# carkod/binquant

Measured on AMD Instinct MI355X. Metric: symbol-candles/s for full indicator set (14 fp64 columns), higher is better.
Workload: dtype f64; 1 GPU; configs[3]: 100000 symbols x 10000 candles, symbol-sharded over 1 GPU(s) (100000 symbols x 10000 candles on rank 0); symbols=100000, symbols_per_gpu=100000, candles=10000, parallelism=symbol-sharded x1, no data-path collective

## Files before the change

binquant_amd/csrc/bq_enrich.hip:

```cpp
#include "bq_device.h"
#include "binquant_amd.h"

#include <stddef.h>
#include <string.h>

#include <type_traits>

namespace bq {

#ifndef BQ_EN_NT
#define BQ_EN_NT 256
#endif
#ifndef BQ_EN_K
#define BQ_EN_K 4
#endif
#ifndef BQ_EN_NTSTORE
#define BQ_EN_NTSTORE 1
#endif
#ifndef BQ_EN_SWIZZLE
#define BQ_EN_SWIZZLE 0
#endif
#ifndef BQ_EN_WPS
#define BQ_EN_WPS 3
#endif
constexpr int EN_NT = BQ_EN_NT;
constexpr int EN_NW = EN_NT / WAVE;
constexpr int EN_K = BQ_EN_K;
constexpr int EN_TT = EN_NT * EN_K;
constexpr int EN_LK = EN_K == 2 ? 1 : EN_K == 4 ? 2 : 3;
constexpr int EN_H = 128;
constexpr int EN_R = EN_H + EN_TT;
static_assert(EN_K % 2 == 0 && EN_TT >= EN_H && EN_K * WAVE > BQ_MAX_WINDOW, "tile shape");

#ifndef BQ_EN_LDSPERM
#define BQ_EN_LDSPERM 1
#endif
#if BQ_EN_LDSPERM
#define LX(i) ((((i) & (EN_K - 1)) * (EN_R / EN_K)) + ((i) >> EN_LK))
#define RS(x) (lb + LX(x))
#define RS1(x) (pb / EN_K + LX(x))
#else
#define LX(i) (i)
#define RS(x) (pb + (x))
#define RS1(x) (pb + (x))
#endif
static_assert(!BQ_EN_LDSPERM || ((1 << EN_LK) == EN_K && EN_R % EN_K == 0), "LX: power-of-two candles per lane");

enum { E_FAST = 0, E_SLOW, E_SIG, E_0, E_1, NE };

struct Pow {
  double a0, a1, p, q, a2, a3, a4;
};

__host__ __device__ __forceinline__ Pow pow_mul(const Pow& T, const Pow& U) {
  Pow r;
  r.a0 = T.a0 * U.a0;
  r.a1 = T.a1 * U.a1;
  r.p = fma(T.p, U.a0, T.a2 * U.p);
  r.q = fma(T.q, U.a1, T.a2 * U.q);
  r.a2 = T.a2 * U.a2;
  r.a3 = T.a3 * U.a3;
  r.a4 = T.a4 * U.a4;
  return r;
}

struct EmaHost {
  double al[NE], om[NE], den[NE], la[NE], lb[NE];
  Pow step;
  Pow wstep[6];
  Pow wave[EN_NW + 1];
};

struct EnrichArgs {
  EmaHost ema;
  const double* in[BQ_NUM_INPUTS];
  double* out[BQ_NUM_ENRICH_COLS];
  int64_t ld_in, ld_out;
  int64_t S, swz;
  int T;
  int ma[3];
  int rsi_w, bb_w, bb_ddof, atr_w, twap_w, mfi_w;
  int span[NE];
  double bb_k;
  double inv_ma[3], inv_rsi, inv_bb, inv_bb_dv, inv_atr, inv_twap;
};

struct EmaConsts {
  double al[NE], om[NE], den[NE], la[NE], lb[NE];
  Pow step;
  Pow wstep[6];
  Pow wave[EN_NW + 1];
  Pow lane[WAVE];
};
static_assert(sizeof(EmaHost) % sizeof(double) == 0 && offsetof(EmaConsts, lane) == sizeof(EmaHost),
              "EmaConsts begins with EmaHost's layout");

static EmaHost ema_consts(const int (&span)[NE]) {
  EmaHost E;
  for (int e = 0; e < NE; ++e) {
    const double com = ((double)span[e] - 1.0) / 2.0;
    const double al = 1.0 / (1.0 + com);
    E.al[e] = al;
    E.om[e] = 1.0 - al;
    E.den[e] = E.om[e] + al;
    E.la[e] = E.om[e] / E.den[e];
    E.lb[e] = al / E.den[e];
  }
  Pow m;
  m.a0 = E.la[E_FAST];
  m.a1 = E.la[E_SLOW];
  m.a2 = E.la[E_SIG];
  m.p = E.lb[E_SIG] * E.la[E_FAST];
  m.q = -(E.lb[E_SIG] * E.la[E_SLOW]);
  m.a3 = E.la[E_0];
  m.a4 = E.la[E_1];
  E.step = m;
  Pow mk = m;
  for (int k = 1; k < EN_K; ++k) mk = pow_mul(m, mk);
  for (int j = 0; j < 6; ++j) {
    E.wstep[j] = mk;
    mk = pow_mul(mk, mk);
  }
  Pow r = {1.0, 1.0, 0.0, 0.0, 1.0, 1.0, 1.0};
  const Pow w64 = pow_mul(E.wstep[5], E.wstep[5]);
  for (int k = 0; k <= EN_NW; ++k) {
    E.wave[k] = r;
    r = pow_mul(w64, r);
  }
  return E;
}

__device__ __forceinline__ void pow_apply(const Pow& A, const double (&v)[NE], double (&r)[NE]) {
  r[E_FAST] = A.a0 * v[E_FAST];
  r[E_SLOW] = A.a1 * v[E_SLOW];
  r[E_SIG] = fma(A.p, v[E_FAST], fma(A.q, v[E_SLOW], A.a2 * v[E_SIG]));
  r[E_0] = A.a3 * v[E_0];
  r[E_1] = A.a4 * v[E_1];
}

template <bool DIV>
__device__ __forceinline__ double ema_step(double y, double x, const EmaConsts& E, int e) {
  if (y != x) {
    y = E.om[e] * y + E.al[e] * x;
    if (DIV) y = y / E.den[e];
  }
  return y;
}

typedef double dbl2 __attribute__((ext_vector_type(2)));

__device__ __forceinline__ void load4(const double* __restrict__ row, int tb, int T, bool vec, double (&x)[EN_K]) {
  if (vec && tb + EN_K <= T) {
    const dbl2* p = reinterpret_cast<const dbl2*>(row + tb);
#pragma unroll
    for (int j = 0; j < EN_K / 2; ++j) {
      const dbl2 a = p[j];
      x[2 * j] = a.x;
      x[2 * j + 1] = a.y;
    }
  } else {
#pragma unroll
    for (int k = 0; k < EN_K; ++k) x[k] = (tb + k < T) ? row[tb + k] : 0.0;
  }
}

typedef __attribute__((address_space(1))) double gdouble;
typedef __attribute__((address_space(1))) dbl2 gdbl2;

#ifndef BQ_EN_SWAPST
#define BQ_EN_SWAPST 1
#endif

__device__ __forceinline__ void put2(gdouble* row, int t, int T, bool full, dbl2 v) {
  if (full || t + 2 <= T) {
#if BQ_EN_NTSTORE
    __builtin_nontemporal_store(v, reinterpret_cast<gdbl2*>(row + t));
#else
    *reinterpret_cast<gdbl2*>(row + t) = v;
#endif
  } else if (t < T) {
    row[t] = v.x;
  }
}

__device__ __forceinline__ void store4(double* __restrict__ row_, int tb, int T, bool vec, const double (&x)[EN_K],
                                       bool full = false) {
  gdouble* row = (gdouble*)row_;
#if BQ_EN_SWAPST
  if constexpr (EN_K == 4) {
    if (vec) {
      union {
        dbl2 d;
        unsigned u[4];
      } a, b;
      a.d = dbl2{x[0], x[1]};
      b.d = dbl2{x[2], x[3]};
#pragma unroll
      for (int i = 0; i < 4; ++i) {
        const auto r = __builtin_amdgcn_permlane32_swap(a.u[i], b.u[i], false, false);
        a.u[i] = r[0];
        b.u[i] = r[1];
      }
      const int lane = __lane_id();
      const int ta = lane < 32 ? tb : tb - 126;
      put2(row, ta, T, full, a.d);
      put2(row, ta + 128, T, full, b.d);
      return;
    }
  }
#endif
  if (vec && tb + EN_K <= T) {
    gdbl2* p = reinterpret_cast<gdbl2*>(row + tb);
#pragma unroll
    for (int j = 0; j < EN_K / 2; ++j) {
#if BQ_EN_NTSTORE
      __builtin_nontemporal_store(dbl2{x[2 * j], x[2 * j + 1]}, p + j);
#else
      p[j] = dbl2{x[2 * j], x[2 * j + 1]};
#endif
    }
  } else {
#pragma unroll
    for (int k = 0; k < EN_K; ++k)
      if (tb + k < T) row[tb + k] = x[k];
  }
}

struct Tile {
  double o[EN_K], h[EN_K], l[EN_K], c[EN_K], v[EN_K];
  double ph, pl, pc;
};

#ifndef BQ_EN_LINELOAD
#define BQ_EN_LINELOAD 0
#endif

__device__ __forceinline__ void load_tile(const EnrichArgs& A, int64_t row, int tb, bool vin, Tile& t) {
  const int T = A.T;
  if (BQ_EN_LINELOAD && vin) {
    load_pieces<EN_K>(A.in[BQ_OPEN] + row, tb, T, t.o, 0.0);
    load_pieces<EN_K>(A.in[BQ_HIGH] + row, tb, T, t.h, 0.0);
    load_pieces<EN_K>(A.in[BQ_LOW] + row, tb, T, t.l, 0.0);
    load_pieces<EN_K>(A.in[BQ_CLOSE] + row, tb, T, t.c, 0.0);
    load_pieces<EN_K>(A.in[BQ_VOLUME] + row, tb, T, t.v, 0.0);
  } else {
    load4(A.in[BQ_OPEN] + row, tb, T, vin, t.o);
    load4(A.in[BQ_HIGH] + row, tb, T, vin, t.h);
    load4(A.in[BQ_LOW] + row, tb, T, vin, t.l);
    load4(A.in[BQ_CLOSE] + row, tb, T, vin, t.c);
    load4(A.in[BQ_VOLUME] + row, tb, T, vin, t.v);
  }
  if (tb >= 1 && tb <= T) {
    t.ph = A.in[BQ_HIGH][row + tb - 1];
    t.pl = A.in[BQ_LOW][row + tb - 1];
    t.pc = A.in[BQ_CLOSE][row + tb - 1];
  } else {
    t.ph = t.pl = t.pc = qnan();
  }
}

__device__ __forceinline__ void tile_arrived(bool vin, Tile& t) {
  if (BQ_EN_LINELOAD && vin) {
    line_unexchange_x<EN_K>(t.o);
    line_unexchange_x<EN_K>(t.h);
    line_unexchange_x<EN_K>(t.l);
    line_unexchange_x<EN_K>(t.c);
    line_unexchange_x<EN_K>(t.v);
  }
}

typedef dbl2 __attribute__((aligned(8))) dbl2u;

__device__ __forceinline__ void load_tile_clamped(const EnrichArgs& A, int64_t row, int tb, Tile& t) {
  const int T = A.T;
  int64_t u[EN_K / 2];
#pragma unroll
  for (int j = 0; j < EN_K / 2; ++j) u[j] = row + min(tb + 2 * j, T - 2);
  auto field = [&](const double* __restrict__ f, double (&x)[EN_K]) {
#pragma unroll
    for (int j = 0; j < EN_K / 2; ++j) {
      const dbl2u a = *reinterpret_cast<const dbl2u*>(f + u[j]);
      x[2 * j] = a.x;
      x[2 * j + 1] = a.y;
    }
  };
  field(A.in[BQ_OPEN], t.o);
  field(A.in[BQ_HIGH], t.h);
  field(A.in[BQ_LOW], t.l);
  field(A.in[BQ_CLOSE], t.c);
  field(A.in[BQ_VOLUME], t.v);
  const int64_t n = row + min(tb - 1, T - 1);
  t.ph = A.in[BQ_HIGH][n];
  t.pl = A.in[BQ_LOW][n];
  t.pc = A.in[BQ_CLOSE][n];
}

__device__ __forceinline__ void tile_tail_select(int tb, int T, Tile& t) {
  auto field = [&](double (&x)[EN_K]) {
#pragma unroll
    for (int j = 0; j < EN_K / 2; ++j) {
      const int u = tb + 2 * j;
      const bool both = u + 2 <= T, one = u < T;
      x[2 * j] = both ? x[2 * j] : (one ? x[2 * j + 1] : 0.0);
      x[2 * j + 1] = both ? x[2 * j + 1] : 0.0;
    }
  };
  field(t.o);
  field(t.h);
  field(t.l);
  field(t.c);
  field(t.v);
  if (tb > T) t.ph = t.pl = t.pc = qnan();
}

template <bool GEN_, bool WARM_, bool RANGE_, bool PREF_, bool SEL_>
struct TileMode {
  static constexpr bool GEN = GEN_, WARM = WARM_, RANGE = RANGE_, PREF = PREF_, SEL = SEL_;
};

template <bool DEF>
__device__ __forceinline__ int win_of(int def, int v) {
  return DEF ? def : __builtin_amdgcn_readfirstlane(v);
}

struct WinAgg {
  double sum, first;
  bool ok, same;
};

template <typename F>
__device__ __forceinline__ WinAgg win_agg(F val, int t, int w) {
  WinAgg a = {0.0, 0.0, t >= w - 1, true};
  if (!a.ok) return a;
  a.first = val(t - w + 1);
  for (int j = t - w + 1; j <= t; ++j) {
    const double x = val(j);
    if (!__builtin_isfinite(x)) {
      a.ok = false;
      return a;
    }
    a.same &= x == a.first;
    a.sum += x;
  }
  return a;
}

__device__ __forceinline__ double ewm_gap_step(double& wt, double& old, double x, double al, double om) {
  const bool obs = __builtin_isfinite(x);
  if (wt == wt) {
    old *= om;
    if (obs) {
      if (wt != x) {
        wt = old * wt + al * x;
        wt /= (old + al);
      }
      old = 1.0;
    }
  } else if (obs) {
    wt = x;
  }
  return wt;
}

__device__ __forceinline__ void enrich_row_missing(const EnrichArgs& P, const EmaConsts& E, int64_t irow, int64_t orow,
                                                double* bc, double* b0, double* b1, double* b2, double* b3) {
  const int tid = threadIdx.x, T = P.T;
  const double* __restrict__ po = P.in[BQ_OPEN] + irow;
  const double* __restrict__ ph = P.in[BQ_HIGH] + irow;
  const double* __restrict__ pl = P.in[BQ_LOW] + irow;
  const double* __restrict__ pc = P.in[BQ_CLOSE] + irow;
  const double* __restrict__ pv = P.in[BQ_VOLUME] + irow;
  auto C = [&](int j) { return j >= 0 ? pc[j] : qnan(); };
  auto TP = [&](int j) { return j >= 0 ? typical_price(ph[j], pl[j], pc[j]) : qnan(); };
  auto put = [&](int col, int t, double v) {
    if (P.out[col]) P.out[col][orow + t] = v;
  };
  auto mean_of = [&](const WinAgg& a, int w) { return !a.ok ? qnan() : (a.same ? a.first : a.sum / (double)w); };
  for (int t = tid; t < T; t += EN_NT) {
    for (int i = 0; i < 3; ++i)
      if (P.out[BQ_MA_FAST + i]) put(BQ_MA_FAST + i, t, mean_of(win_agg(C, t, P.ma[i]), P.ma[i]));
    if (P.out[BQ_BB_UPPER] || P.out[BQ_BB_MID] || P.out[BQ_BB_LOWER]) {
      const int w = P.bb_w;
      const WinAgg a = win_agg(C, t, w);
      double m = qnan(), sd = qnan();
      if (a.ok) {
        m = mean_of(a, w);
        double ss = 0.0;
        if (!a.same)
          for (int j = t - w + 1; j <= t; ++j) {
            const double d = pc[j] - m;
            ss += d * d;
          }
        sd = w - P.bb_ddof > 0 ? sqrt(ss / (double)(w - P.bb_ddof)) : qnan();
      }
      put(BQ_BB_MID, t, m);
      put(BQ_BB_UPPER, t, m + (P.bb_k * sd));
      put(BQ_BB_LOWER, t, m - (P.bb_k * sd));
    }
    if (P.out[BQ_TWAP])
      put(BQ_TWAP, t, mean_of(win_agg([&](int j) { return ohlc4(po[j], ph[j], pl[j], pc[j]); }, t, P.twap_w),
                              P.twap_w));
    if (P.out[BQ_ATR])
      put(BQ_ATR, t, mean_of(win_agg([&](int j) { return true_range(ph[j], pl[j], C(j - 1)); }, t, P.atr_w),
                             P.atr_w));
    if (P.out[BQ_RSI]) {
      const int w = P.rsi_w;
      const WinAgg g = win_agg([&](int j) { const double d = C(j) - C(j - 1); return d > 0.0 ? d : 0.0; }, t, w);
      const WinAgg l = win_agg([&](int j) { const double d = C(j) - C(j - 1); return d < 0.0 ? -d : 0.0; }, t, w);
      const double rs = mean_of(g, w) / mean_of(l, w);
      put(BQ_RSI, t, 100.0 - (100.0 / (1.0 + rs)));
    }
    if (P.out[BQ_MFI]) {
      const int w = P.mfi_w;
      const WinAgg p = win_agg([&](int j) { const double tp = TP(j); return tp > TP(j - 1) ? tp * pv[j] : 0.0; }, t, w);
      const WinAgg n = win_agg([&](int j) { const double tp = TP(j); return tp < TP(j - 1) ? tp * pv[j] : 0.0; }, t, w);
      const double ps = p.ok ? p.sum : qnan(), ns = n.ok ? n.sum : qnan();
      put(BQ_MFI, t, 100.0 - (100.0 / (1.0 + ps / ns)));
    }
  }
  const bool ema = P.out[BQ_MACD] || P.out[BQ_MACD_SIGNAL] || P.out[BQ_EMA_FAST] || P.out[BQ_EMA_SLOW];
  if (!ema) return;
  double wf = qnan(), of = 1.0, ws = qnan(), os = 1.0, wg = qnan(), og = 1.0, we = qnan(), oe = 1.0;
  for (int c0 = 0; c0 < T; c0 += EN_TT) {
    const int n = min(EN_TT, T - c0);
    __syncthreads();
    for (int i = tid; i < n; i += EN_NT) bc[i] = pc[c0 + i];
    __syncthreads();
    if (tid == 0) {
      for (int i = 0; i < n; ++i) {
        const double x = bc[i];
        const double f = ewm_gap_step(wf, of, x, E.al[E_FAST], E.om[E_FAST]);
        const double s = ewm_gap_step(ws, os, x, E.al[E_SLOW], E.om[E_SLOW]);
        const double m = f - s;
        b0[i] = m;
        b1[i] = ewm_gap_step(wg, og, m, E.al[E_SIG], E.om[E_SIG]);
      }
    } else if (tid == WAVE || tid == 2 * WAVE) {
      const int e = tid == WAVE ? E_0 : E_1;
      double* dst = tid == WAVE ? b2 : b3;
      for (int i = 0; i < n; ++i) dst[i] = ewm_gap_step(we, oe, bc[i], E.al[e], E.om[e]);
    }
    __syncthreads();
    for (int i = tid; i < n; i += EN_NT) {
      put(BQ_MACD, c0 + i, b0[i]);
      put(BQ_MACD_SIGNAL, c0 + i, b1[i]);
      put(BQ_EMA_FAST, c0 + i, b2[i]);
      put(BQ_EMA_SLOW, c0 + i, b3[i]);
    }
  }
}

template <bool DIV, bool VOUT, bool DEF, bool HOT = false>
__global__ __launch_bounds__(EN_NT, BQ_EN_WPS) void enrich_kernel(const EnrichArgs A, int vec_in) {
  static_assert(!HOT || (!DIV && VOUT && DEF && !BQ_EN_LINELOAD && EN_K == 4), "HOT: the common call only");
  __shared__ double sP[EN_R];
  __shared__ double sC[EN_R];
  __shared__ double sTR[EN_R];
  __shared__ double sO4[EN_R];
  __shared__ double sMF[EN_R];
  __shared__ double sWh[EN_NW], sWl[EN_NW];
  __shared__ double sWe[EN_NW][NE];
  __shared__ int sWlc[EN_NW];
  __shared__ double sEcar[NE];
  __shared__ int sLcar, sMiss;
  __shared__ EmaConsts E;
  __shared__ EnrichArgs sA;

  const int tid = threadIdx.x, lane = tid & (WAVE - 1), w = tid / WAVE;
  const int64_t sym = BQ_EN_SWIZZLE ? ((int64_t)blockIdx.x * A.swz) % A.S : (int64_t)blockIdx.x;
  const int64_t irow = sym * A.ld_in;
  const int64_t orow = sym * A.ld_out;
  const int T = A.T;
  const bool vin = HOT || vec_in != 0, vout = VOUT;

  Tile nx;
  load_tile(A, irow, EN_K * tid, vin, nx);

  {
    const double* src = reinterpret_cast<const double*>(&A.ema);
    double* dst = reinterpret_cast<double*>(&E);
    for (int i = tid; i < (int)(sizeof(EmaHost) / sizeof(double)); i += EN_NT) dst[i] = src[i];
  }
  if (tid < WAVE) {
    Pow r = {1.0, 1.0, 0.0, 0.0, 1.0, 1.0, 1.0};
    for (int j = 0; j < 6; ++j)
      if (tid & (1 << j)) r = pow_mul(A.ema.wstep[j], r);
    E.lane[tid] = r;
  }
  if (tid < NE) sEcar[tid] = 0.0;
  if (tid == 0) {
    sLcar = -1;
    sMiss = 0;
    sA = A;
  }
  if (tid < EN_H) {
    sP[LX(tid)] = 0.0;
    sC[LX(tid)] = qnan();
    sTR[LX(tid)] = 0.0;
    sO4[LX(tid)] = 0.0;
    sMF[LX(tid)] = 0.0;
  }
  __syncthreads();

  if (tid == 0) {
    const double x0 = nx.c[0];
    sEcar[E_FAST] = sEcar[E_SLOW] = sEcar[E_0] = sEcar[E_1] = x0;
    sEcar[E_SIG] = 0.0;
  }

  const int pb = EN_H + EN_K * tid;
  int lcl[EN_K];
  double Ploc[EN_K];
  double y[NE];
  auto ploc = [&](int k) -> double {
    if constexpr (HOT) return sP[RS1(k)];
    else return Ploc[k];
  };

  auto tile = [&](auto mode, const int t0) {
    using M = decltype(mode);
    const int tb = t0 + EN_K * tid;
    const EnrichArgs& P = sA;
    auto has = [&](int col) { return HOT || P.out[col] != nullptr; };
    Tile cu = nx;
    if constexpr (M::SEL) tile_tail_select(tb, T, cu);
    else tile_arrived(vin, cu);
    if constexpr (M::GEN) {
      if (t0 + EN_TT < T) load_tile(A, irow, tb + EN_TT, vin, nx);
    }

    {
      bool miss = false;
      double pc = cu.pc;
      double tpp = typical_price(cu.ph, cu.pl, cu.pc);
      int run = -1;
#pragma unroll
      for (int k = 0; k < EN_K; ++k) {
        const int t = tb + k;
        const double c = cu.c[k];
        const double tp = typical_price(cu.h[k], cu.l[k], c);
        const double mf = tp * cu.v[k];
        const double o4 = ohlc4(cu.o[k], cu.h[k], cu.l[k], c);
        miss |= !__builtin_isfinite(o4) | !__builtin_isfinite(mf);
        sC[RS1(k)] = c;
        sTR[RS1(k)] = true_range(cu.h[k], cu.l[k], pc);
        sO4[RS1(k)] = o4;
        sMF[RS1(k)] = tp > tpp ? mf : (tp < tpp ? -mf : 0.0);
        if (t == 0 || c != pc) run = t;
        lcl[k] = run;
        pc = c;
        tpp = tp;
      }
      if (__builtin_amdgcn_ballot_w64(miss)) sMiss = 1;
    }
    if constexpr (M::PREF) load_tile_clamped(A, irow, tb + EN_TT, nx);
    {
      dd tot = {0.0, 0.0};
#pragma unroll
      for (int k = 0; k < EN_K; ++k) tot = dd_add1(tot, cu.c[k]);
      const dd inc = wave_scan_dd_dpp(tot, lane);
      if (lane == WAVE - 1) {
        sWh[w] = inc.hi;
        sWl[w] = inc.lo;
      }
      dd acc = {dpp_f64<DPP_WAVE_SHR1>(inc.hi), dpp_f64<DPP_WAVE_SHR1>(inc.lo)};
#pragma unroll
      for (int k = 0; k < EN_K; ++k) {
        acc = dd_add1(acc, cu.c[k]);
        Ploc[k] = dd_round(acc);
        sP[RS1(k)] = Ploc[k];
      }
    }
    double ex[NE];
    {
      double b[NE] = {0.0, 0.0, 0.0, 0.0, 0.0};
#pragma unroll
      for (int k = 0; k < EN_K; ++k) {
        const double x = cu.c[k];
        b[E_FAST] = fma(E.la[E_FAST], b[E_FAST], E.lb[E_FAST] * x);
        b[E_SLOW] = fma(E.la[E_SLOW], b[E_SLOW], E.lb[E_SLOW] * x);
        b[E_SIG] = fma(E.la[E_SIG], b[E_SIG], E.lb[E_SIG] * (b[E_FAST] - b[E_SLOW]));
        b[E_0] = fma(E.la[E_0], b[E_0], E.lb[E_0] * x);
        b[E_1] = fma(E.la[E_1], b[E_1], E.lb[E_1] * x);
      }
#define BQ_EMA_STEP(CTRL, J)                                     \
  {                                                              \
    double v[NE], r[NE];                                         \
    _Pragma("unroll") for (int e = 0; e < NE; ++e) v[e] = dpp_f64<CTRL>(b[e]); \
    pow_apply(E.wstep[J], v, r);                                 \
    _Pragma("unroll") for (int e = 0; e < NE; ++e) b[e] += r[e]; \
  }
      BQ_EMA_STEP(DPP_ROW_SHR1, 0)
      BQ_EMA_STEP(DPP_ROW_SHR2, 1)
      BQ_EMA_STEP(DPP_ROW_SHR4, 2)
      BQ_EMA_STEP(DPP_ROW_SHR8, 3)
#undef BQ_EMA_STEP
      {
        double c1[NE], c2[NE], c3[NE], r[NE];
#pragma unroll
        for (int e = 0; e < NE; ++e) c1[e] = readlane_f64(b[e], 15);
        pow_apply(E.wstep[4], c1, r);
#pragma unroll
        for (int e = 0; e < NE; ++e) c2[e] = r[e] + readlane_f64(b[e], 31);
        pow_apply(E.wstep[4], c2, r);
#pragma unroll
        for (int e = 0; e < NE; ++e) c3[e] = r[e] + readlane_f64(b[e], 47);
        const int row = lane >> 4;
        if (row > 0) {
          double c[NE];
#pragma unroll
          for (int e = 0; e < NE; ++e) c[e] = row == 1 ? c1[e] : (row == 2 ? c2[e] : c3[e]);
          pow_apply(E.lane[(lane & 15) + 1], c, r);
#pragma unroll
          for (int e = 0; e < NE; ++e) b[e] += r[e];
        }
      }
      if (lane == WAVE - 1) {
#pragma unroll
        for (int e = 0; e < NE; ++e) sWe[w][e] = b[e];
      }
#pragma unroll
      for (int e = 0; e < NE; ++e) ex[e] = dpp_f64<DPP_WAVE_SHR1>(b[e]);
    }
    int lpre;
    {
      const int inc = wave_scan_max_dpp(lcl[EN_K - 1] + 1, lane);
      if (lane == WAVE - 1) sWlc[w] = inc - 1;
      lpre = dpp_i32<DPP_WAVE_SHR1>(inc) - 1;
    }
    __syncthreads();

    double wb[EN_NW];
    {
      dd acc = {0.0, 0.0};
#pragma unroll
      for (int u = 0; u < EN_NW; ++u) {
        wb[u] = dd_round(acc);
        acc = dd_add(acc, dd{sWh[u], sWl[u]});
      }
    }
    {
      int carry = max(sLcar, lpre);
      for (int u = 0; u < w; ++u) carry = max(carry, sWlc[u]);
#pragma unroll
      for (int k = 0; k < EN_K; ++k) lcl[k] = max(lcl[k], carry);
    }
    {
      double C[NE];
#pragma unroll
      for (int e = 0; e < NE; ++e) C[e] = sEcar[e];
      for (int u = 0; u < w; ++u) {
        double r[NE];
        pow_apply(E.wave[1], C, r);
#pragma unroll
        for (int e = 0; e < NE; ++e) C[e] = r[e] + sWe[u][e];
      }
      double r[NE];
      pow_apply(E.lane[lane], C, r);
#pragma unroll
      for (int e = 0; e < NE; ++e) y[e] = ex[e] + r[e];
    }

    {
      double mfast[EN_K], msig[EN_K], e0[EN_K], e1[EN_K];
#pragma unroll
      for (int k = 0; k < EN_K; ++k) {
        const double x = cu.c[k];
        y[E_FAST] = ema_step<DIV>(y[E_FAST], x, E, E_FAST);
        y[E_SLOW] = ema_step<DIV>(y[E_SLOW], x, E, E_SLOW);
        y[E_SIG] = ema_step<DIV>(y[E_SIG], y[E_FAST] - y[E_SLOW], E, E_SIG);
        y[E_0] = ema_step<DIV>(y[E_0], x, E, E_0);
        y[E_1] = ema_step<DIV>(y[E_1], x, E, E_1);
        mfast[k] = y[E_FAST] - y[E_SLOW];
        msig[k] = y[E_SIG];
        e0[k] = y[E_0];
        e1[k] = y[E_1];
      }
      const bool whole = M::GEN ? t0 + EN_TT <= T : !M::RANGE;
      if (has(BQ_MACD)) store4(P.out[BQ_MACD] + orow, tb, T, vout, mfast, whole);
      if (has(BQ_MACD_SIGNAL)) store4(P.out[BQ_MACD_SIGNAL] + orow, tb, T, vout, msig, whole);
      if (has(BQ_EMA_FAST)) store4(P.out[BQ_EMA_FAST] + orow, tb, T, vout, e0, whole);
      if (has(BQ_EMA_SLOW)) store4(P.out[BQ_EMA_SLOW] + orow, tb, T, vout, e1, whole);
    }

    double wbw = wb[0], wbp = 0.0;
#pragma unroll
    for (int u = 1; u < EN_NW; ++u) {
      if (w == u) {
        wbw = wb[u];
        wbp = wb[u - 1];
      }
    }
    const int wstart = EN_H + EN_K * WAVE * w;
    auto windows = [&](auto nowarmc, auto fullstc) {
      constexpr bool NOWARM = decltype(nowarmc)::value;
      constexpr bool FULLST = decltype(fullstc)::value;
      const int gstart = EN_H - t0;
      const int lb = pb / EN_K;
      (void)lb;
      auto warm = [&](int t, int win) { return !NOWARM && t < win - 1; };
      auto put = [&](double* col, const double (&x)[EN_K]) {
        if (FULLST) store4(col + orow, tb, T, true, x, true);
        else store4(col + orow, tb, T, vout, x);
      };
      auto cmean = [&](int win, double inv, int k) -> double {
        const int t = tb + k, p = pb + k;
        if (warm(t, win)) return qnan();
        if (lcl[k] <= t - win + 1) return cu.c[k];
        const int q = p - win;
        const double base = q >= wstart ? wbw : wbp;
        return div_exact((ploc(k) + wbw) - (sP[RS(k - win)] + base), (double)win, inv);
      };
      double res[EN_K];
#pragma unroll
      for (int i = 0; i < 3; ++i) {
        if (has(BQ_MA_FAST + i)) {
          const int win = win_of<DEF>(i == 0 ? 7 : (i == 1 ? 25 : 100), P.ma[i]);
          const double inv = P.inv_ma[i];
#pragma unroll
          for (int k = 0; k < EN_K; ++k) res[k] = cmean(win, inv, k);
          put(P.out[BQ_MA_FAST + i], res);
        }
      }
      if (has(BQ_BB_UPPER) || has(BQ_BB_MID) || has(BQ_BB_LOWER)) {
        double up[EN_K], mid[EN_K], lo[EN_K];
        const int win = win_of<DEF>(20, P.bb_w);
        const double bk = P.bb_k, invw = P.inv_bb, invdv = P.inv_bb_dv;
        const bool okdv = win > P.bb_ddof;
        const double r = cu.c[0];
        double s1 = 0.0, s2 = 0.0;
        walk_window<DEF && NOWARM>(NOWARM ? 1 - win : max(1 - win, gstart - pb), [&](int x) {
          const double d = sC[RS(x)] - r;
          s1 += d;
          s2 = fma(d, d, s2);
        });
#pragma unroll
        for (int k = 0; k < EN_K; ++k) {
          const int t = tb + k, p = pb + k;
          if (k > 0) {
            const double dn = cu.c[k] - r;
            const double dol = (NOWARM || p - win >= gstart) ? sC[RS(k - win)] - r : 0.0;
            s1 = (s1 + dn) - dol;
            s2 = fma(-dol, dol, fma(dn, dn, s2));
          }
          const double m = cmean(win, invw, k);
          double sd;
          if (warm(t, win) || !okdv) sd = qnan();
          else if (lcl[k] <= t - win + 1) sd = 0.0;
          else {
            const double var = (s2 - s1 * s1 * invw) * invdv;
            sd = sqrt_nr(var);
          }
          mid[k] = m;
          up[k] = m + bk * sd;
          lo[k] = m - bk * sd;
        }
        if (has(BQ_BB_UPPER)) put(P.out[BQ_BB_UPPER], up);
        if (has(BQ_BB_MID)) put(P.out[BQ_BB_MID], mid);
        if (has(BQ_BB_LOWER)) put(P.out[BQ_BB_LOWER], lo);
      }
      if (has(BQ_RSI)) {
        const int win = win_of<DEF>(14, P.rsi_w);
        double A = 0.0, prev = sC[RS(-win)];
        int nup = 0, ndn = 0;
        walk_window<DEF>(1 - win, [&](int x) {
          const double c = sC[RS(x)], d = c - prev;
          A += fmax(fabs(d), 0.0);
          nup += d > 0.0;
          ndn += d < 0.0;
          prev = c;
        });
#pragma unroll
        for (int k = 0; k < EN_K; ++k) {
          const int t = tb + k, p = pb + k;
          if (k > 0) {
            const double d = cu.c[k] - cu.c[k - 1];
            const double dold = sC[RS(k - win)] - sC[RS(k - win - 1)];
            A = (A + fabs(d)) - fmax(fabs(dold), 0.0);
            nup += (d > 0.0) - (dold > 0.0);
            ndn += (d < 0.0) - (dold < 0.0);
          }
          if (warm(t, win)) {
            res[k] = qnan();
            continue;
          }
          const double D = cu.c[k] - sC[NOWARM ? RS(k - win) : (p - win >= gstart ? RS(k - win) : LX(gstart))];
          double v;
          if (nup == 0 && ndn == 0) v = qnan();
          else if (ndn == 0) v = 100.0;
          else if (nup == 0) v = 0.0;
          else v = 50.0 * (1.0 + D / A);
          res[k] = v;
        }
        put(P.out[BQ_RSI], res);
      }
      auto smean = [&](const double* Q, int defw, int win_, double inv, bool nonneg) {
        const int win = win_of<DEF>(defw, win_);
        const double wd = (double)win;
        double sum = 0.0, pq = qnan();
        int run = 0;
        walk_window<DEF>(1 - win, [&](int x) {
          const double q = Q[RS(x)];
          sum += q;
          run = q == pq ? run + 1 : 1;
          pq = q;
        });
#pragma unroll
        for (int k = 0; k < EN_K; ++k) {
          const int t = tb + k;
          if (k > 0) {
            const double q = Q[RS(k)];
            sum = (sum + q) - Q[RS(k - win)];
            run = q == pq ? run + 1 : 1;
            pq = q;
          }
          if (warm(t, win)) res[k] = qnan();
          else if (run >= win) res[k] = pq;
          else res[k] = div_exact(nonneg && sum < 0.0 ? 0.0 : sum, wd, inv);
        }
      };
      if (has(BQ_ATR)) {
        smean(sTR, 14, P.atr_w, P.inv_atr, true);
        put(P.out[BQ_ATR], res);
      }
      if (has(BQ_TWAP)) {
        smean(sO4, 12, P.twap_w, P.inv_twap, false);
        put(P.out[BQ_TWAP], res);
      }
      if (has(BQ_MFI)) {
        const int win = win_of<DEF>(14, P.mfi_w);
        double B = 0.0, F = 0.0;
        int nup = 0, ndn = 0;
        walk_window<DEF>(1 - win, [&](int x) {
          const double f = sMF[RS(x)];
          B += fabs(f);
          F += f;
          nup += f > 0.0;
          ndn += f < 0.0;
        });
#pragma unroll
        for (int k = 0; k < EN_K; ++k) {
          const int t = tb + k;
          if (k > 0) {
            const double f = sMF[RS(k)], fo = sMF[RS(k - win)];
            B = (B + fabs(f)) - fabs(fo);
            F = (F + f) - fo;
            nup += (f > 0.0) - (fo > 0.0);
            ndn += (f < 0.0) - (fo < 0.0);
          }
          double v;
          if (warm(t, win) || (nup == 0 && ndn == 0)) v = qnan();
          else if (ndn == 0) v = 100.0;
          else if (nup == 0) v = 0.0;
          else v = 50.0 * (1.0 + F / B);
          res[k] = v;
        }
        put(P.out[BQ_MFI], res);
      }
    };
    if constexpr (M::GEN) {
      const bool full = t0 >= EN_H && t0 + EN_TT <= T && vout;
      if (full) windows(std::true_type{}, std::true_type{});
      else windows(std::false_type{}, std::false_type{});
    } else {
      windows(std::bool_constant<!M::WARM>{}, std::bool_constant<!M::RANGE>{});
    }
  };

  auto halo = [&]() {
    __syncthreads();
    const double plast = HOT ? sP[LX(EN_R - 1)] : __shfl(Ploc[EN_K - 1], WAVE - 1, WAVE);
    if (pb >= EN_TT) {
#pragma unroll
      for (int k = 0; k < EN_K; ++k) {
        sP[RS1(k - EN_TT)] = ploc(k) - plast;
        sC[RS1(k - EN_TT)] = sC[RS1(k)];
        sTR[RS1(k - EN_TT)] = sTR[RS1(k)];
        sO4[RS1(k - EN_TT)] = sO4[RS1(k)];
        sMF[RS1(k - EN_TT)] = sMF[RS1(k)];
      }
    }
    if (tid == EN_NT - 1) {
#pragma unroll
      for (int e = 0; e < NE; ++e) sEcar[e] = y[e];
      sLcar = lcl[EN_K - 1];
    }
  };

  if constexpr (!HOT) {
    for (int t0 = 0; t0 < T; t0 += EN_TT) {
      tile(TileMode<true, false, false, false, false>{}, t0);
      if (t0 + EN_TT >= T) break;
      halo();
    }
  } else if (T < EN_TT) {
    tile(TileMode<false, true, true, false, false>{}, 0);
  } else {
    tile(TileMode<false, true, false, true, false>{}, 0);
    int t0 = EN_TT;
    for (; t0 + EN_TT <= T; t0 += EN_TT) {
      halo();
      tile(TileMode<false, false, false, true, false>{}, t0);
    }
    if (t0 < T) {
      halo();
      tile(TileMode<false, false, true, false, true>{}, t0);
    }
  }
  __syncthreads();
  if (sMiss) enrich_row_missing(sA, E, irow, orow, sC, sP, sTR, sO4, sMF);
}

static bool window_ok(int w) { return w >= 1 && w <= BQ_MAX_WINDOW; }

}

extern "C" {

void bq_default_params(bq_params* p) {
  if (!p) return;
  memset(p, 0, sizeof(*p));
  p->ma_periods[0] = 7;
  p->ma_periods[1] = 25;
  p->ma_periods[2] = 100;
  p->macd_fast = 12;
  p->macd_slow = 26;
  p->macd_signal = 9;
  p->rsi_window = 14;
  p->bb_window = 20;
  p->bb_ddof = 1;
  p->atr_window = 14;
  p->twap_window = 12;
  p->ema_spans[0] = 20;
  p->ema_spans[1] = 50;
  p->mfi_window = 14;
  p->bb_k = 2.0;
}

const char* bq_version(void) { return "binquant_amd 0.2.0 (gfx950)"; }

int bq_device_arch(char* buf, int buflen) {
  if (!buf || buflen <= 0) return BQ_EINVAL;
  int dev = 0;
  if (hipGetDevice(&dev) != hipSuccess) return BQ_EHIP;
  hipDeviceProp_t prop;
  if (hipGetDeviceProperties(&prop, dev) != hipSuccess) return BQ_EHIP;
  strncpy(buf, prop.gcnArchName, (size_t)buflen - 1);
  buf[buflen - 1] = 0;
  return BQ_OK;
}

int bq_enrich(const double* const* in, int64_t S, int64_t T, int64_t ld_in, const bq_params* params,
              double* const* out, int64_t ld_out, void* stream) {
  using namespace bq;
  if (!in || !out || S < 0 || T < 0 || ld_in < T || ld_out < T || T > (int64_t)0x7fffffff - 2 * EN_TT ||
      S > 0x7fffffff)
    return BQ_EINVAL;
  bq_params dp;
  if (!params) {
    bq_default_params(&dp);
    params = &dp;
  }
  const bq_params& P = *params;
  for (int i = 0; i < 3; ++i)
    if (!window_ok(P.ma_periods[i])) return BQ_EINVAL;
  if (!window_ok(P.rsi_window) || !window_ok(P.bb_window) || !window_ok(P.atr_window) ||
      !window_ok(P.twap_window) || !window_ok(P.mfi_window) || P.bb_ddof < 0 || P.macd_fast < 1 ||
      P.macd_slow < 1 || P.macd_signal < 1 || P.ema_spans[0] < 1 || P.ema_spans[1] < 1)
    return BQ_EINVAL;
  EnrichArgs A;
  memset(&A, 0, sizeof(A));
  bool any_out = false;
  for (int i = 0; i < BQ_NUM_INPUTS; ++i) {
    if (!in[i]) return BQ_EINVAL;
    A.in[i] = in[i];
  }
  for (int i = 0; i < BQ_NUM_ENRICH_COLS; ++i) {
    A.out[i] = out[i];
    any_out |= out[i] != nullptr;
  }
  if (S == 0 || T == 0 || !any_out) return BQ_OK;
  A.ld_in = ld_in;
  A.ld_out = ld_out;
  A.T = (int)T;
  A.S = S;
  A.swz = 1;
  {
    auto gcd = [](int64_t a, int64_t b) {
      while (b) {
        const int64_t t = a % b;
        a = b;
        b = t;
      }
      return a;
    };
    const int64_t primes[] = {7919, 7927, 7933, 7937, 7949, 104729};
    for (int64_t p : primes)
      if (S > 1 && gcd(p % S, S) == 1) {
        A.swz = p % S;
        break;
      }
  }
  for (int i = 0; i < 3; ++i) A.ma[i] = P.ma_periods[i];
  A.rsi_w = P.rsi_window;
  A.bb_w = P.bb_window;
  A.bb_ddof = P.bb_ddof;
  A.atr_w = P.atr_window;
  A.twap_w = P.twap_window;
  A.mfi_w = P.mfi_window;
  A.bb_k = P.bb_k;
  for (int i = 0; i < 3; ++i) A.inv_ma[i] = 1.0 / (double)P.ma_periods[i];
  A.inv_rsi = 1.0 / (double)P.rsi_window;
  A.inv_bb = 1.0 / (double)P.bb_window;
  A.inv_bb_dv = P.bb_window > P.bb_ddof ? 1.0 / (double)(P.bb_window - P.bb_ddof) : 0.0;
  A.inv_atr = 1.0 / (double)P.atr_window;
  A.inv_twap = 1.0 / (double)P.twap_window;
  A.span[E_FAST] = P.macd_fast;
  A.span[E_SLOW] = P.macd_slow;
  A.span[E_SIG] = P.macd_signal;
  A.span[E_0] = P.ema_spans[0];
  A.span[E_1] = P.ema_spans[1];
  A.ema = ema_consts(A.span);

  auto aligned = [](const void* p) { return (((uintptr_t)p) & 15u) == 0; };
  int vin = (ld_in % 2) == 0;
  for (int i = 0; i < BQ_NUM_INPUTS; ++i) vin &= aligned(in[i]);
  int vout = (ld_out % 2) == 0;
  for (int i = 0; i < BQ_NUM_ENRICH_COLS; ++i)
    if (out[i]) vout &= aligned(out[i]);

  bool div = false;
  for (int e = 0; e < NE; ++e) {
    const double com = ((double)A.span[e] - 1.0) / 2.0;
    const double al = 1.0 / (1.0 + com);
    div |= ((1.0 - al) + al) != 1.0;
  }
  const dim3 grid((unsigned)S), block(EN_NT);
  hipStream_t st = (hipStream_t)stream;
  const bool def = P.ma_periods[0] == 7 && P.ma_periods[1] == 25 && P.ma_periods[2] == 100 && P.rsi_window == 14 &&
                   P.bb_window == 20 && P.atr_window == 14 && P.twap_window == 12 && P.mfi_window == 14;
  bool hot = def && !div && vout && vin && !BQ_EN_LINELOAD && EN_K == 4;
  for (int i = 0; i < BQ_NUM_ENRICH_COLS; ++i) hot &= out[i] != nullptr;
#define BQ_EN_LAUNCH(D, V, F) hipLaunchKernelGGL((enrich_kernel<D, V, F>), grid, block, 0, st, A, vin)
  if (hot) {
    if constexpr (!BQ_EN_LINELOAD && EN_K == 4)
      hipLaunchKernelGGL((enrich_kernel<false, true, true, true>), grid, block, 0, st, A, vin);
  } else if (def) {
    if (div && vout) BQ_EN_LAUNCH(true, true, true);
    else if (div) BQ_EN_LAUNCH(true, false, true);
    else if (vout) BQ_EN_LAUNCH(false, true, true);
    else BQ_EN_LAUNCH(false, false, true);
  } else {
    if (div && vout) BQ_EN_LAUNCH(true, true, false);
    else if (div) BQ_EN_LAUNCH(true, false, false);
    else if (vout) BQ_EN_LAUNCH(false, true, false);
    else BQ_EN_LAUNCH(false, false, false);
  }
#undef BQ_EN_LAUNCH
  return hipGetLastError() == hipSuccess ? BQ_OK : BQ_EHIP;
}

}
```

Measured before the change: 37.35 billion symbol-candles/s.

## Branchless selects, uniform wave index, and double-buffered EMA carry in hot enrich kernel

Replaces divergent branches in the EMA step, lane-row fixup, rolling-mean, Bollinger, RSI and MFI paths with computed-then-selected values. It makes the wave index scalar-uniform via readfirstlane and fully unrolls the per-wave carry loops. The EMA carry is double-buffered through the last wave's sWe slot so the carry write no longer needs to wait for the halo phase. Halo copies are batched as all loads then all stores. The cost is extra arithmetic on lanes that previously skipped work, and some added complexity in the parity-based carry buffer handling.

After: 38.44 billion symbol-candles/s (median of 6 runs). +2.9%, better.

```diff
diff --git a/binquant_amd/csrc/bq_enrich.hip b/binquant_amd/csrc/bq_enrich.hip
--- a/binquant_amd/csrc/bq_enrich.hip
+++ b/binquant_amd/csrc/bq_enrich.hip
@@ -138,16 +138,28 @@
   r[E_1] = A.a4 * v[E_1];
 }
 
-template <bool DIV>
+template <bool DIV, bool SEL = false>
 __device__ __forceinline__ double ema_step(double y, double x, const EmaConsts& E, int e) {
-  if (y != x) {
-    y = E.om[e] * y + E.al[e] * x;
-    if (DIV) y = y / E.den[e];
-  }
-  return y;
+  static_assert(!(DIV && SEL), "SEL: without the divide only");
+  if constexpr (SEL) {
+    const double n = E.om[e] * y + E.al[e] * x;
+    return y != x ? n : y;
+  } else {
+    if (y != x) {
+      y = E.om[e] * y + E.al[e] * x;
+      if (DIV) y = y / E.den[e];
+    }
+    return y;
+  }
 }
 
 typedef double dbl2 __attribute__((ext_vector_type(2)));
+
+__device__ __forceinline__ double sel_f64(bool c, double a, double b) {
+  const int hi = c ? __double2hiint(a) : __double2hiint(b);
+  const int lo = c ? __double2loint(a) : __double2loint(b);
+  return __hiloint2double(hi, lo);
+}
 
 __device__ __forceinline__ void load4(const double* __restrict__ row, int tb, int T, bool vec, double (&x)[EN_K]) {
   if (vec && tb + EN_K <= T) {
@@ -466,7 +478,8 @@
   __shared__ EmaConsts E;
   __shared__ EnrichArgs sA;
 
-  const int tid = threadIdx.x, lane = tid & (WAVE - 1), w = tid / WAVE;
+  const int tid = threadIdx.x, lane = tid & (WAVE - 1);
+  const int w = __builtin_amdgcn_readfirstlane(tid / WAVE);
   const int64_t sym = BQ_EN_SWIZZLE ? ((int64_t)blockIdx.x * A.swz) % A.S : (int64_t)blockIdx.x;
   const int64_t irow = sym * A.ld_in;
   const int64_t orow = sym * A.ld_out;
@@ -516,6 +529,11 @@
     if constexpr (HOT) return sP[RS1(k)];
     else return Ploc[k];
   };
+
+  constexpr bool DBUF = HOT;
+  int par = 0;
+  auto ecar_in = [&]() -> const double* { return DBUF && par ? sWe[EN_NW - 1] : sEcar; };
+  auto ecar_out = [&]() -> double* { return par ? sEcar : sWe[EN_NW - 1]; };
 
   auto tile = [&](auto mode, const int t0) {
     using M = decltype(mode);
@@ -606,16 +624,17 @@
 #pragma unroll
         for (int e = 0; e < NE; ++e) c3[e] = r[e] + readlane_f64(b[e], 47);
         const int row = lane >> 4;
-        if (row > 0) {
-          double c[NE];
-#pragma unroll
-          for (int e = 0; e < NE; ++e) c[e] = row == 1 ? c1[e] : (row == 2 ? c2[e] : c3[e]);
-          pow_apply(E.lane[(lane & 15) + 1], c, r);
-#pragma unroll
-          for (int e = 0; e < NE; ++e) b[e] += r[e];
+        double c[NE];
+#pragma unroll
+        for (int e = 0; e < NE; ++e) {
+          const double a1 = c1[e], a2 = c2[e], a3 = c3[e];
+          c[e] = row == 1 ? a1 : (row == 2 ? a2 : a3);
         }
-      }
-      if (lane == WAVE - 1) {
+        pow_apply(E.lane[(lane & 15) + 1], c, r);
+#pragma unroll
+        for (int e = 0; e < NE; ++e) b[e] = sel_f64(row > 0, b[e] + r[e], b[e]);
+      }
+      if (lane == WAVE - 1 && (!DBUF || w < EN_NW - 1)) {
 #pragma unroll
         for (int e = 0; e < NE; ++e) sWe[w][e] = b[e];
       }
@@ -630,30 +649,40 @@
     }
     __syncthreads();
 
-    double wb[EN_NW];
+    double wbw = 0.0, wbp = 0.0;
     {
       dd acc = {0.0, 0.0};
 #pragma unroll
       for (int u = 0; u < EN_NW; ++u) {
-        wb[u] = dd_round(acc);
-        acc = dd_add(acc, dd{sWh[u], sWl[u]});
+        const double base = dd_round(acc);
+        wbw = u == w ? base : wbw;
+        wbp = u + 1 == w ? base : wbp;
+        if (u + 1 < EN_NW) acc = dd_add(acc, dd{sWh[u], sWl[u]});
       }
     }
     {
       int carry = max(sLcar, lpre);
-      for (int u = 0; u < w; ++u) carry = max(carry, sWlc[u]);
+      int wl[EN_NW - 1];
+#pragma unroll
+      for (int u = 0; u < EN_NW - 1; ++u) wl[u] = sWlc[u];
+#pragma unroll
+      for (int u = 0; u < EN_NW - 1; ++u) carry = u < w ? max(carry, wl[u]) : carry;
 #pragma unroll
       for (int k = 0; k < EN_K; ++k) lcl[k] = max(lcl[k], carry);
     }
     {
       double C[NE];
 #pragma unroll
-      for (int e = 0; e < NE; ++e) C[e] = sEcar[e];
-      for (int u = 0; u < w; ++u) {
-        double r[NE];
-        pow_apply(E.wave[1], C, r);
-#pragma unroll
-        for (int e = 0; e < NE; ++e) C[e] = r[e] + sWe[u][e];
+      for (int e = 0; e < NE; ++e) C[e] = ecar_in()[e];
+      const Pow W1 = E.wave[1];
+#pragma unroll
+      for (int u = 0; u < EN_NW - 1; ++u) {
+        if (u < w) {
+          double r[NE];
+          pow_apply(W1, C, r);
+#pragma unroll
+          for (int e = 0; e < NE; ++e) C[e] = r[e] + sWe[u][e];
+        }
       }
       double r[NE];
       pow_apply(E.lane[lane], C, r);
@@ -666,15 +695,21 @@
 #pragma unroll
       for (int k = 0; k < EN_K; ++k) {
         const double x = cu.c[k];
-        y[E_FAST] = ema_step<DIV>(y[E_FAST], x, E, E_FAST);
-        y[E_SLOW] = ema_step<DIV>(y[E_SLOW], x, E, E_SLOW);
-        y[E_SIG] = ema_step<DIV>(y[E_SIG], y[E_FAST] - y[E_SLOW], E, E_SIG);
-        y[E_0] = ema_step<DIV>(y[E_0], x, E, E_0);
-        y[E_1] = ema_step<DIV>(y[E_1], x, E, E_1);
+        y[E_FAST] = ema_step<DIV, HOT>(y[E_FAST], x, E, E_FAST);
+        y[E_SLOW] = ema_step<DIV, HOT>(y[E_SLOW], x, E, E_SLOW);
+        y[E_SIG] = ema_step<DIV, HOT>(y[E_SIG], y[E_FAST] - y[E_SLOW], E, E_SIG);
+        y[E_0] = ema_step<DIV, HOT>(y[E_0], x, E, E_0);
+        y[E_1] = ema_step<DIV, HOT>(y[E_1], x, E, E_1);
         mfast[k] = y[E_FAST] - y[E_SLOW];
         msig[k] = y[E_SIG];
         e0[k] = y[E_0];
         e1[k] = y[E_1];
+      }
+      if constexpr (DBUF) {
+        if (tid == EN_NT - 1) {
+#pragma unroll
+          for (int e = 0; e < NE; ++e) ecar_out()[e] = y[e];
+        }
       }
       const bool whole = M::GEN ? t0 + EN_TT <= T : !M::RANGE;
       if (has(BQ_MACD)) store4(P.out[BQ_MACD] + orow, tb, T, vout, mfast, whole);
@@ -683,20 +718,13 @@
       if (has(BQ_EMA_SLOW)) store4(P.out[BQ_EMA_SLOW] + orow, tb, T, vout, e1, whole);
     }
 
-    double wbw = wb[0], wbp = 0.0;
-#pragma unroll
-    for (int u = 1; u < EN_NW; ++u) {
-      if (w == u) {
-        wbw = wb[u];
-        wbp = wb[u - 1];
-      }
-    }
     const int wstart = EN_H + EN_K * WAVE * w;
     auto windows = [&](auto nowarmc, auto fullstc) {
       constexpr bool NOWARM = decltype(nowarmc)::value;
       constexpr bool FULLST = decltype(fullstc)::value;
       const int gstart = EN_H - t0;
-      const int lb = pb / EN_K;
+      int lb = pb / EN_K;
+      if constexpr (HOT) asm volatile("" : "+v"(lb));
       (void)lb;
       auto warm = [&](int t, int win) { return !NOWARM && t < win - 1; };
       auto put = [&](double* col, const double (&x)[EN_K]) {
@@ -705,11 +733,11 @@
       };
       auto cmean = [&](int win, double inv, int k) -> double {
         const int t = tb + k, p = pb + k;
-        if (warm(t, win)) return qnan();
-        if (lcl[k] <= t - win + 1) return cu.c[k];
         const int q = p - win;
         const double base = q >= wstart ? wbw : wbp;
-        return div_exact((ploc(k) + wbw) - (sP[RS(k - win)] + base), (double)win, inv);
+        const double m = div_exact((ploc(k) + wbw) - (sP[RS(k - win)] + base), (double)win, inv);
+        const double v = lcl[k] <= t - win + 1 ? cu.c[k] : m;
+        return warm(t, win) ? qnan() : v;
       };
       double res[EN_K];
 #pragma unroll
@@ -739,18 +767,15 @@
           const int t = tb + k, p = pb + k;
           if (k > 0) {
             const double dn = cu.c[k] - r;
-            const double dol = (NOWARM || p - win >= gstart) ? sC[RS(k - win)] - r : 0.0;
+            const double cold = sC[RS(k - win)];
+            const double dol = (NOWARM || p - win >= gstart) ? cold - r : 0.0;
             s1 = (s1 + dn) - dol;
             s2 = fma(-dol, dol, fma(dn, dn, s2));
           }
           const double m = cmean(win, invw, k);
-          double sd;
-          if (warm(t, win) || !okdv) sd = qnan();
-          else if (lcl[k] <= t - win + 1) sd = 0.0;
-          else {
-            const double var = (s2 - s1 * s1 * invw) * invdv;
-            sd = sqrt_nr(var);
-          }
+          const double var = (s2 - s1 * s1 * invw) * invdv;
+          const double sdv = lcl[k] <= t - win + 1 ? 0.0 : sqrt_nr(var);
+          const double sd = (warm(t, win) || !okdv) ? qnan() : sdv;
           mid[k] = m;
           up[k] = m + bk * sd;
           lo[k] = m - bk * sd;
@@ -780,17 +805,12 @@
             nup += (d > 0.0) - (dold > 0.0);
             ndn += (d < 0.0) - (dold < 0.0);
           }
-          if (warm(t, win)) {
-            res[k] = qnan();
-            continue;
-          }
           const double D = cu.c[k] - sC[NOWARM ? RS(k - win) : (p - win >= gstart ? RS(k - win) : LX(gstart))];
-          double v;
-          if (nup == 0 && ndn == 0) v = qnan();
-          else if (ndn == 0) v = 100.0;
-          else if (nup == 0) v = 0.0;
-          else v = 50.0 * (1.0 + D / A);
-          res[k] = v;
+          double v = 50.0 * (1.0 + D / A);
+          v = nup == 0 ? 0.0 : v;
+          v = ndn == 0 ? 100.0 : v;
+          v = (nup == 0 && ndn == 0) ? qnan() : v;
+          res[k] = warm(t, win) ? qnan() : v;
         }
         put(P.out[BQ_RSI], res);
       }
@@ -814,9 +834,9 @@
             run = q == pq ? run + 1 : 1;
             pq = q;
           }
-          if (warm(t, win)) res[k] = qnan();
-          else if (run >= win) res[k] = pq;
-          else res[k] = div_exact(nonneg && sum < 0.0 ? 0.0 : sum, wd, inv);
+          const double m = div_exact(nonneg && sum < 0.0 ? 0.0 : sum, wd, inv);
+          const double v = run >= win ? pq : m;
+          res[k] = warm(t, win) ? qnan() : v;
         }
       };
       if (has(BQ_ATR)) {
@@ -848,12 +868,10 @@
             nup += (f > 0.0) - (fo > 0.0);
             ndn += (f < 0.0) - (fo < 0.0);
           }
-          double v;
-          if (warm(t, win) || (nup == 0 && ndn == 0)) v = qnan();
-          else if (ndn == 0) v = 100.0;
-          else if (nup == 0) v = 0.0;
-          else v = 50.0 * (1.0 + F / B);
-          res[k] = v;
+          double v = 50.0 * (1.0 + F / B);
+          v = nup == 0 ? 0.0 : v;
+          v = ndn == 0 ? 100.0 : v;
+          res[k] = (warm(t, win) || (nup == 0 && ndn == 0)) ? qnan() : v;
         }
         put(P.out[BQ_MFI], res);
       }
@@ -871,20 +889,32 @@
     __syncthreads();
     const double plast = HOT ? sP[LX(EN_R - 1)] : __shfl(Ploc[EN_K - 1], WAVE - 1, WAVE);
     if (pb >= EN_TT) {
+      double hp[EN_K], hc[EN_K], htr[EN_K], ho4[EN_K], hmf[EN_K];
 #pragma unroll
       for (int k = 0; k < EN_K; ++k) {
-        sP[RS1(k - EN_TT)] = ploc(k) - plast;
-        sC[RS1(k - EN_TT)] = sC[RS1(k)];
-        sTR[RS1(k - EN_TT)] = sTR[RS1(k)];
-        sO4[RS1(k - EN_TT)] = sO4[RS1(k)];
-        sMF[RS1(k - EN_TT)] = sMF[RS1(k)];
+        hp[k] = ploc(k) - plast;
+        hc[k] = sC[RS1(k)];
+        htr[k] = sTR[RS1(k)];
+        ho4[k] = sO4[RS1(k)];
+        hmf[k] = sMF[RS1(k)];
+      }
+#pragma unroll
+      for (int k = 0; k < EN_K; ++k) {
+        sP[RS1(k - EN_TT)] = hp[k];
+        sC[RS1(k - EN_TT)] = hc[k];
+        sTR[RS1(k - EN_TT)] = htr[k];
+        sO4[RS1(k - EN_TT)] = ho4[k];
+        sMF[RS1(k - EN_TT)] = hmf[k];
       }
     }
     if (tid == EN_NT - 1) {
-#pragma unroll
-      for (int e = 0; e < NE; ++e) sEcar[e] = y[e];
+      if constexpr (!DBUF) {
+#pragma unroll
+        for (int e = 0; e < NE; ++e) sEcar[e] = y[e];
+      }
       sLcar = lcl[EN_K - 1];
     }
+    if constexpr (DBUF) par ^= 1;
   };
 
   if constexpr (!HOT) {
```
